# HyeonwooNoh/VQA-Transfer-ExternalData

Measured on AMD Instinct MI355X. Metric: VQA train samples/sec (img+question) at bs512, higher is better.
Workload: dtype f32

## Files before the change

### include/vqa_hot.h

```cpp
#ifndef VQA_HOT_H
#define VQA_HOT_H

#include <stdint.h>

#ifdef __cplusplus
extern "C" {
#endif

#define VQA_HOT_ABI_VERSION 5

enum {
    VQA_OK = 0,
    VQA_ERR_ARG = -1,
    VQA_ERR_ALIGN = -2,
    VQA_ERR_LAUNCH = -3,
    VQA_ERR_UNSUPPORTED = -4,
    VQA_ERR_WORKSPACE = -5
};

int vqa_hot_version(void);
const char* vqa_hot_error_string(int code);

int vqa_gather_features(const float* table, const int32_t* nbox_table, const int64_t* idx,
                        float* V, int32_t* nb, int B, int R, int D, int64_t N, void* stream);
// ... 291 lines not shown
    vqa_fc_t v2l[3];
    vqa_fc_t answer_layer1, pooled_layer1, q_layer1;
    vqa_fc_t classifier;
} vqa_params_t;

typedef struct {
    const float* table;
    const int32_t* nbox_table;
    const int64_t* image_idx;
    const int32_t* q_intseq;
    const int32_t* q_intseq_len;
    const float* answer_target;
    const float *train_mask, *obj_mask, *attr_mask, *exist_mask;
    const uint8_t* keep_att;
    const uint8_t* keep_joint;
    const uint8_t* keep_joint2;
    const int32_t* live_rows;
    const float* noise;
    const uint8_t* keep_tile;
    const uint8_t* keep_word;
    const int32_t* answer_intseq;
    const int32_t* answer_intseq_len;
    uint64_t keep_seed;
    uint64_t keep_att_off, keep_joint_off, keep_joint2_off, keep_tile_off, keep_word_off;
    int32_t keep_seeded;
} vqa_batch_t;
#define VQA_KEEP_SITE_ATT 1
#define VQA_KEEP_SITE_JOINT 2
#define VQA_KEEP_SITE_JOINT2 4
#define VQA_KEEP_SITE_TILE 8
#define VQA_KEEP_SITE_WORD 16

int64_t vqa_fusion_workspace_bytes(const vqa_dims_t* dims);
int vqa_fusion_tensor(const vqa_dims_t* dims, const char* name, int64_t* offset_bytes, int64_t* n_elems);
int vqa_fusion_forward(const vqa_dims_t* dims, const vqa_params_t* params, const vqa_batch_t* batch,
                       void* workspace, int64_t workspace_bytes, int want_dz, void* stream);
int vqa_fusion_backward(const vqa_dims_t* dims, const vqa_params_t* params, const vqa_params_t* grads,
                        const vqa_batch_t* batch, void* workspace, int64_t workspace_bytes,
                        float* embed_slice_sq, void* stream);

typedef struct {
    int32_t B, n, R, D, H, W, A, Vq, n_ws;
    int32_t L;
    int32_t flags;
    float keep_att, keep_joint;
    float global_valid[2];
} vqa_pretrain_dims_t;

typedef struct { float *w, *b, *beta[4], *gamma[4]; } vqa_pt_fc_t;

typedef struct {
    float* wordset_map;
    float* l_glove;
    vqa_pt_fc_t spat_v_linear_v;
    vqa_pt_fc_t spat_q_linear_v;
    vqa_pt_fc_t spat_att_score;
    float *gru_wg, *gru_bg, *gru_wc, *gru_bc;
    vqa_pt_fc_t pooled_linear_l;
    vqa_pt_fc_t q_linear_l;
    vqa_pt_fc_t joint_fc;
    vqa_pt_fc_t wordset_ft;
    vqa_pt_fc_t classifier;
} vqa_pretrain_params_t;

typedef struct {
    const float* normal_boxes;
// ... 290 lines not shown
```

### vqa-transfer-externaldata_amd/_lib.py

```python
from __future__ import annotations

import ctypes as C
import os

_HERE = os.path.dirname(os.path.abspath(__file__))
_LIB_PATH = os.path.join(_HERE, "libvqahot.so")


class VqaHotError(RuntimeError):
    pass


def lib_path():
    return _LIB_PATH


class Dims(C.Structure):
    _fields_ = [("B", C.c_int32), ("R", C.c_int32), ("D", C.c_int32), ("H", C.c_int32), ("T", C.c_int32),
                ("W", C.c_int32), ("A", C.c_int32), ("Vq", C.c_int32), ("N_img", C.c_int64),
                ("model_type", C.c_int32), ("keep_att", C.c_float), ("keep_joint", C.c_float),
                ("inv_global_batch", C.c_float), ("flags", C.c_int32),
                ("num_marginal", C.c_int32), ("ent_cols", C.c_int32), ("extra_weight", C.c_float),
                ("map_dim", C.c_int32), ("La", C.c_int32)]

# ... 184 lines not shown
    "vqa_ln_relu_bwd": (_I, [_P, _P, _P, _P, _P, _P, _P, _F, _P, _P, _P, _P, _I, _I, _I, _P]),
    "vqa_ln_act_fwd": (_I, [_P, _P, _P, _P, _F, _P, _P, _P, _I, _I, _I, _I, _P]),
    "vqa_ln_act_bwd": (_I, [_P, _P, _P, _P, _P, _P, _P, _F, _P, _P, _P, _P, _I, _I, _I, _I, _P]),
    "vqa_ln_pair_mul_supported": (_I, [_I, _P, _I]),
    "vqa_ln_pair_mul_fwd": (_I, [_P] * 13 + [_I, _I, _P]),
    "vqa_ln_pair_mul_bwd": (_I, [_P] * 20 + [_I, _I, _P]),
    "vqa_tanh_fwd": (_I, [_P, _P, _L, _P]),
    "vqa_tanh_bwd": (_I, [_P, _P, _P, _L, _P]),
    "vqa_softmax_ce_fwd": (_I, [_P, _P, _P, _I, _P, _P, _P, _I, _I, _P]),
    "vqa_softmax_set_fast": (_I, [_I]),
    "vqa_softmax_ce_pair_fwd": (_I, [C.POINTER(SoftmaxPair), _I, _I, _I, _I, _P]),
    "vqa_colsum": (_I, [_P, _I, _I, _I, _P, _P, _L, _P]),
    "vqa_colsum_workspace_floats": (_L, [_I, _I]),
    "vqa_colsum3": (_I, [_P, _P, _P, _I, _I, _I, _P, _P, _P, _P, _L, _P]),
    "vqa_colsum_acc": (_I, [_P, _I, _I, _I, _P, _I, _P, _L, _P]),
    "vqa_colsum3_acc": (_I, [_P, _P, _P, _I, _I, _I, _P, _P, _P, _I, _P, _L, _P]),
    "vqa_mul": (_I, [_P, _P, _P, _L, _P]),
    "vqa_mul_bwd": (_I, [_P, _P, _P, _P, _P, _L, _P]),
    "vqa_add_inplace": (_I, [_P, _P, _L, _P]),
    "vqa_gru_gates_fwd": (_I, [_P, _I, _P, _P, _P, _P, _I, _I, _P]),
    "vqa_gru_cand_fwd": (_I, [_P, _I, _P, _P, _P, _I, _P, _P, _I, _I, _P]),
    "vqa_gru_bwd_a": (_I, [_P, _P, _P, _P, _P, _I, _P, _I, _P, _I, _P, _I, _I, _P]),
    "vqa_gru_bwd_b": (_I, [_P, _P, _P, _P, _I, _P, _I, _I, _P]),
    "vqa_attn_set_fast": (_I, [_I]),
    "vqa_attn_pool_fwd": (_I, [_P, _P, _P, _P, _P, _P, _P, _F, _P, _P, _I, _I, _I, _I, _P]),
    "vqa_attn_pool_bwd": (_I, [_P, _P, _P, _P, _P, _P, _P, _F, _P, _P, _P, _P, _I, _I, _I, _I, _P]),
    "vqa_attn_pool_fwd_v16": (_I, [_P, _P, _P, _P, _P, _P, _P, _F, _P, _P, _I, _I, _I, _I, _P]),
    "vqa_attn_pool_bwd_v16": (_I, [_P, _P, _P, _P, _P, _P, _P, _F, _P, _P, _P, _P, _I, _I, _I, _I, _P]),
    "vqa_attn_pool_fwd_rep": (_I, [_P, _P, _P, _P, _P, _P, _P, _F, _P, _P, _I, _I, _I, _I, _I, _P]),
    "vqa_attn_pool_bwd_rep": (_I, [_P, _P, _P, _P, _P, _P, _P, _F, _P, _P, _P, _P, _I, _I, _I, _I, _I, _P]),
    "vqa_vtail_supported": (_I, [_I, _I, _I, _I]),
    "vqa_vtail_set_mode": (_I, [_I]),
    "vqa_gru_h0skip_set_mode": (_I, [_I]),
    "vqa_attn_pool_bwd_ds": (_I, [_P, _P, _P, _P, _P, _I, _I, _I, _I, _I, _P]),
    "vqa_attn_pool_bwd_ds_v16": (_I, [_P, _P, _P, _P, _P, _I, _I, _I, _I, _I, _P]),
    "vqa_ln_relu_att_bwd": (_I, [_P, _P, _P, _P, _F] + [_P] * 11 + [_I, _I, _I, _I, _I, _P]),
    "vqa_attn_pool_fwd_seeded": (_I, [_P, _P, _P, _I, _P, _P, _P, _U, _U, _F, _P, _P, _I, _I, _I, _I, _I, _P]),
    "vqa_attn_pool_bwd_seeded": (_I, [_P, _P, _P, _P, _I, _P, _P, _U, _U, _F, _P, _P, _P, _P, _I, _I, _I, _I, _I, _P]),
    "vqa_attn_pool_fwd_rep_seeded": (_I, [_P, _P, _P, _P, _P, _P, _U, _U, _F, _P, _P, _I, _I, _I, _I, _I, _P]),
    "vqa_attn_pool_bwd_rep_seeded": (_I, [_P, _P, _P, _P, _P, _P, _U, _U, _F, _P, _P, _P, _P, _I, _I, _I, _I, _I, _P]),
    "vqa_ln_act_fwd_seeded": (_I, [_P, _P, _P, _U, _U, _F, _P, _P, _P, _I, _I, _I, _I, _P]),
    "vqa_ln_act_bwd_seeded": (_I, [_P, _P, _P, _P, _P, _P, _U, _U, _F, _P, _P, _P, _P, _I, _I, _I, _I, _P]),
    "vqa_ln_relu_att_bwd_seeded": (_I, [_P, _P, _P, _U, _U, _F] + [_P] * 11 + [_I, _I, _I, _I, _I, _P]),
    "vqa_colsum_vtail_workspace_floats": (_L, [_I, _I]),
    "vqa_colsum_vtail": (_I, [_P] * 5 + [_I, _I] + [_P] * 6 + [_L, _P]),
    "vqa_loss_fwd": (_I, [_P, _P, _P, _P, _P, _P, _I, _F, _P, _P, _P, _I, _I, _P]),
    "vqa_loss2_fwd": (_I, [_P, _P, _P, _P, _P, _P, _P, _F, _P, _P, _P, _P, _P, _I, _I, _I, _P]),
    "vqa_rowmin_mask_fwd": (_I, [_P, _P, _P, _P, _I, _I, _P]),
    "vqa_rowmin_mask_bwd": (_I, [_P, _P, _P, _P, _I, _I, _P]),
    "vqa_report_reduce": (_I, [_P, _I, _P, _P]),
    "vqa_report_key": (C.c_char_p, [_I]),
    "vqa_sumsq": (_I, [_P, _L, _P, _P, _P, _L, _P]),
    "vqa_sumsq_workspace_floats": (_L, [_L]),
    "vqa_clip_adam": (_I, [_P, _P, _P, _P, _L, _P, _F, _F, _F, _F, _F, _P]),
    "vqa_dropout_mask": (_I, [_P, _L, C.c_uint64, C.c_uint64, _F, _P]),
    "vqa_clip_adam_dev": (_I, [_P, _P, _P, _P, _L, _P, _F, _P, _F, _F, _F, _P]),
    "vqa_embed2_fwd": (_I, [_P, _P, _P, _P, _I, _I, _I, _I, _P]),
    "vqa_embed2_bwd": (_I, [_P, _P, _P, _P, _I, _I, _I, _I, _P]),
    "vqa_lstm_step_fwd": (_I, [_P, _P, _P, _P, _I, _P, _P, _I, _I, _P]),
    "vqa_lstm_step_bwd": (_I, [_P, _P, _P, _P, _P, _P, _I, _P, _P, _P, _I, _I, _P]),
    "vqa_relu_fwd": (_I, [_P, _P, _L, _P]),
    "vqa_relu_bwd": (_I, [_P, _P, _P, _L, _P]),
    "vqa_fill": (_I, [_P, _L, _F, _P]),
    "vqa_score_fwd": (_I, [_P, _P, _P, _P, _P, _I, _I, _I, _P]),
    "vqa_score_bwd": (_I, [_P, _P, _P, _P, _P, _P, _P, _I, _I, _I, _P]),
    "vqa_reverse_tokens": (_I, [_P, _P, _P, _I, _I, _P]),
# ... 131 lines not shown
```

### vqa-transfer-externaldata_amd/csrc/fusion_model.hip

```cpp
#include <stdlib.h>
#include <string.h>

#include <string>
#include <vector>

#include "keep_launch.h"

namespace {

struct Entry { const char* name; int64_t off; int64_t n; int esz; };

struct Layout {
    std::vector<Entry> e;
    int64_t total = 0;
    int64_t add(const char* name, int64_t n, int esz = 4) {
        const int64_t off = total;
        e.push_back({name, off, n, esz});
        total += ((n * esz + 255) / 256) * 256;
        return off;
    }
    const Entry* find(const char* name) const {
        for (const auto& x : e)
            if (strcmp(x.name, name) == 0) return &x;
        return nullptr;
    }
};

inline bool has_tuned_head(int mt) { return mt == VQA_MODEL_VQA_ALL2 || mt == VQA_MODEL_VQA_ALL; }
inline bool train_loss_masked(int mt) { return mt != VQA_MODEL_STANDARD; }
inline bool bf16_routed(int mt) { return mt == VQA_MODEL_VLMAP_ANSWER || mt == VQA_MODEL_STANDARD; }
inline bool feat16(const vqa_dims_t& d) { return (d.flags & VQA_FLAG_BF16_FEATURES) != 0; }

void legacy_vqa_layout(Layout& L, const vqa_dims_t& d, int64_t& gw);

Layout make_layout(const vqa_dims_t& d) {
    Layout L;
    const int64_t B = d.B, R = d.R, D = d.D, H = d.H, T = d.T, W = d.W, A = d.A;
    L.add("V_ft", B * R * D, feat16(d) ? 2 : 4);
// ... 151 lines not shown
    int64_t colsum_ws_floats() const { return L.find("colsum_ws")->n; }
};

inline bool env_on(const char* name, bool dflt) {
    const char* e = getenv(name);
    return e == nullptr ? dflt : atoi(e) != 0;
}
inline bool xcat_enabled() { static const bool v = env_on("VQA_HOT_XCAT", true); return v; }
inline bool repack_enabled() { static const bool v = env_on("VQA_HOT_REPACK", false); return v; }
inline bool gru_ws_on() { static const bool v = env_on("VQA_HOT_GRU_WS", true); return v; }
inline bool visual_late_enabled() { static const bool v = env_on("VQA_HOT_VISUAL_LATE", true); return v; }
inline bool ln_pair_enabled() { static const bool v = env_on("VQA_HOT_LN_PAIR", true); return v; }
int g_vtail_mode = -1;
inline int vtail_mode() {
    if (g_vtail_mode < 0) g_vtail_mode = env_on("VQA_HOT_VTAIL", true) ? 1 : 0;
    return g_vtail_mode;
}
int g_h0skip_mode = -1;
inline int h0skip_mode() {
    if (g_h0skip_mode < 0) {
        const char* e = getenv("VQA_HOT_GRU_H0SKIP");
        g_h0skip_mode = e == nullptr ? 1 : (atoi(e) & 3);
    }
    return g_h0skip_mode;
}
int side_max_blocks() {
    static int v = -1;
    if (v < 0) {
        const char* e = getenv("VQA_HOT_SIDE_BLOCKS");
        v = e ? atoi(e) : 0;
    }
    return v;
}
int gather_mode(const vqa_dims_t* dims) {
    static int env = -2;
    if (env == -2) {
        const char* e = getenv("VQA_HOT_GATHER");
        env = e == nullptr ? -1 : (strcmp(e, "fused") == 0 ? 1 : 0);
    }
    if (env >= 0) return env;
    return (dims->flags & VQA_FLAG_FUSED_GATHER) ? 1 : 0;
}

struct Side {
    hipStream_t s = nullptr;
    hipEvent_t fork = nullptr, join = nullptr;
    bool ok = false, tried = false;
};
Side& side_stream() {
    static Side sd[64];
    int dev = 0;
    (void)hipGetDevice(&dev);
    Side& x = sd[dev & 63];
    if (!x.tried) {
        x.tried = true;
        const char* env = getenv("VQA_HOT_OVERLAP");
        if (env != nullptr && env[0] == '1') {
            x.ok = hipStreamCreateWithFlags(&x.s, hipStreamNonBlocking) == hipSuccess &&
                   hipEventCreateWithFlags(&x.fork, hipEventDisableTiming) == hipSuccess &&
                   hipEventCreateWithFlags(&x.join, hipEventDisableTiming) == hipSuccess;
        }
    }
    return x;
}
struct Chains {
    static constexpr int MAXC = 4;
    hipStream_t s[MAXC] = {};
    hipEvent_t fork = nullptr, join[MAXC] = {};
    int n = 1;
    float delay_us = 3.f;
    bool tried = false;
};
Chains& gru_chains() {
    static Chains ch[64];
// ... 321 lines not shown

extern "C" int vqa_fusion_tensor(const vqa_dims_t* dims, const char* name, int64_t* offset_bytes, int64_t* n_elems) {
    if (!dims_ok(dims) || name == nullptr) return VQA_ERR_ARG;
    const Layout L = make_layout(*dims);
    const char* key = name;
    if (strcmp(name, "condition") == 0 && dims->model_type == VQA_MODEL_ANSWER2) key = "q_L_ft2";
    else if (strcmp(name, "condition") == 0 && dims->model_type == VQA_MODEL_BI) key = "q_L_ft";
    else if (dims->model_type == VQA_MODEL_LEGACY_VQA && (strcmp(name, "q_L_ft") == 0 || strcmp(name, "answer_ft") == 0)) {
        const bool q = name[0] == 'q';
        const Entry* hsn = L.find(q ? "lv_hsq" : "lv_hsa");
        const int64_t N = q ? dims->B : dims->A, Tn = q ? dims->T : dims->La;
        if (offset_bytes) *offset_bytes = hsn->off + Tn * N * dims->H * 4;
        if (n_elems) *n_elems = N * dims->H;
        return VQA_OK;
    }
    else if (strcmp(name, "condition") == 0) {
        const Entry* h = L.find("hs");
        if (offset_bytes) *offset_bytes = h->off + (int64_t)dims->T * dims->B * dims->H * 4;
        if (n_elems) *n_elems = (int64_t)dims->B * dims->H;
        return VQA_OK;
    }
    const Entry* e = L.find(key);
    if (e == nullptr) return VQA_ERR_ARG;
    if (offset_bytes) *offset_bytes = e->off;
    if (n_elems) *n_elems = e->n;
    return VQA_OK;
}

extern "C" int vqa_vtail_set_mode(int mode) {
    g_vtail_mode = mode < 0 ? -1 : (mode ? 1 : 0);
    return vtail_mode();
}

extern "C" int vqa_gru_h0skip_set_mode(int mode) {
    g_h0skip_mode = mode < 0 ? -1 : (mode & 3);
    return h0skip_mode();
}

namespace {

struct Step {
    const vqa_dims_t& d;
    const vqa_params_t* const P;
    const vqa_params_t* const G;
    const vqa_batch_t* const bt;
    const Layout L;
    const Ctx c;
    const int mt;
    const int64_t B, R, D, H, T, W, A;
    const int64_t Wp;
    const int64_t Dp;
    Side* sd = nullptr;
    bool forked = false;
    bool fuse_gather = false, visual_late = false;
    const float* q_ft = nullptr;
    const float* qv_in = nullptr;
    const float* lin_in = nullptr;
    bool pair = false;

    Step(const vqa_dims_t* dims, const vqa_params_t* P_, const vqa_params_t* G_, const vqa_batch_t* bt_, void* workspace,
         void* stream)
        : d(*dims), P(P_), G(G_), bt(bt_), L(make_layout(*dims)),
          c{*dims, L, static_cast<char*>(workspace), static_cast<hipStream_t>(stream), 0}, mt(dims->model_type),
          B(dims->B), R(dims->R), D(dims->D), H(dims->H), T(dims->T), W(dims->W), A(dims->A), Wp(x_stride(dims->W)),
          Dp(pooled_dim(*dims)) {}
    Step(const Step&) = delete;
// ... 2 lines not shown
    Ctx side_ctx() const { return Ctx{d, L, c.ws, forked ? sd->s : c.st, forked ? 1 : 0}; }
    const float* hs = nullptr;
    const float* h = nullptr;
    float* dh = nullptr;
    float* dxp = nullptr;
    void bind_bwd() {
        hs = c.f("hs");
        h = hs + T * B * H;
        dh = c.f("d_h0");
        dxp = c.f("dxp");
    }
    const float* Wg_h() const { return P->gru_wg + W * 2 * H; }
    const float* Wc_h() const { return P->gru_wc + W * H; }
};

int side_record(const Step& s) { return !s.forked || join_side_record(*s.sd) ? VQA_OK : VQA_ERR_LAUNCH; }
int side_wait(const Step& s) {
    return !s.forked || hipStreamWaitEvent(s.c.st, s.sd->join, 0) == hipSuccess ? VQA_OK : VQA_ERR_LAUNCH;
}

enum GruForm { GRU_WS, GRU_LIVE, GRU_CHAINS };
enum GruDir { GRU_FWD, GRU_BWD };
GruForm gru_form(GruDir dir, int64_t T, int64_t B, int64_t H, const int32_t* live_rows) {
    const bool ws_ok = gru_ws_on() && (live_rows == nullptr || (T > 0 && live_rows[T - 1] > 0));
    if (ws_ok && (dir == GRU_FWD ? vqa_gru_ws_supported((int)T, (int)B, (int)H) : vqa_gru_ws_bwd_supported((int)T, (int)B, (int)H)) == 1)
        return GRU_WS;
    return live_rows != nullptr ? GRU_LIVE : GRU_CHAINS;
}


void fwd_visual_plan(Step& s) {
    s.sd = &side_stream();
    s.forked = fork_side(s.c, *s.sd);
    s.fuse_gather = !(s.d.flags & VQA_FLAG_BF16_GEMM) && gather_mode(&s.d) == 1 && (s.D % 32 == 0) && (s.H % 4 == 0) &&
                    vqa_aligned16(s.bt->table);
    s.visual_late = !s.forked && visual_late_enabled();
}

int fwd_visual(const Step& s) {
    const Ctx cv = s.side_ctx();
    const vqa_params_t* P = s.P;
    const vqa_batch_t* bt = s.bt;
    const int64_t B = s.B, R = s.R, D = s.D, H = s.H;
    {
        ProbeScope ps("gather", cv.st);
        if (feat16(s.d))
            TRY(vqa_gather_features_bf16(reinterpret_cast<const uint16_t*>(bt->table), bt->nbox_table, bt->image_idx,
                                         cv.u16("V_ft"), cv.i32("num_V_ft"), (int)B, (int)R, (int)D, s.d.N_img, cv.st));
        else
            TRY(vqa_gather_features(bt->table, bt->nbox_table, bt->image_idx, s.fuse_gather ? nullptr : cv.f("V_ft"),
                                    cv.i32("num_V_ft"), (int)B, (int)R, (int)D, s.d.N_img, cv.st));
    }
    if (s.fuse_gather) {
        {
            ProbeScope ps("v_linear_v.fwd_gemm", cv.st);
            TRY(vqa_gemm_f32_gather((int)(B * R), (int)H, (int)D, bt->table, (int)D, bt->image_idx, (int)R, s.d.N_img,
                                    P->v_linear_v.w, (int)H, cv.f("pre_v"), (int)H, P->v_linear_v.b, cv.f("V_ft"), (int)D,
                                    cv.st));
        }
        ProbeScope ps("v_linear_v.ln_fwd", cv.st);
        TRY(vqa_ln_relu_fwd(cv.f("pre_v"), P->v_linear_v.gamma, P->v_linear_v.beta, nullptr, 1.f, cv.f("v_linear_v"),
                            cv.f("mean_v"), cv.f("rstd_v"), (int)B, (int)R, (int)H, cv.st));
    } else {
        TRY(fc_ln_relu_fwd(cv, cv.f("V_ft"), B * R, D, H, P->v_linear_v, (int)R, "pre_v", "v_linear_v", "mean_v", "rstd_v",
                           NO_KEEP, 1.f));
    }
    if (s.mt == VQA_MODEL_ADAPT) {
        VQA_REQUIRE(P->v_adapt.w != nullptr && P->v_adapt.gamma != nullptr, VQA_ERR_ARG);
// ... 622 lines not shown
```

### vqa-transfer-externaldata_amd/csrc/gemm_args.h

```cpp
#pragma once
#include <hip/hip_runtime.h>
#include <stdint.h>

struct GemmArgs {
    int M, N, K;
    const float* A; int lda;
    const float* B; int ldb;
    float* C; int ldc;
    const float* bias;
    const float* D; int ldd;
    int k_per_split;
    int64_t slab_stride;
    int vecA, vecB;
    int tiles_m, tiles_n, nsplit;
    int m_fastest;
    unsigned a_bytes, b_bytes;
    const float* scale;
    int relu;
    int Hi, Wi, Ci, Ho, Wo, cstride, pad_t, pad_l, kw;
    int conv_taps;
    int vec_epi;
    const int64_t* g_idx; int g_R; int64_t g_N; float* g_out; int g_ldo;
};

enum { EPI_PLAIN = 0, EPI_GATES = 1, EPI_CAND = 2, EPI_BWD_RH = 3, EPI_BWD_DH = 4 };
struct EpiArgs {
    int H, t, ldo;
    const int32_t* len;
    const float* h_prev;
    const float* i0;
    const float* i1;
    float* o0;
    float* o1;
    float* o2;
};

GemmArgs vqa_gemm_make_args(int M, int N, int K, const float* A, int lda, const float* B, int ldb, float* C, int ldc,
                            const float* bias, const float* D, int ldd);
int vqa_gru_step_launch(int epi, int cfg, const GemmArgs& a, const EpiArgs& ep, hipStream_t st);
int vqa_gru_rs_launch(int epi, const GemmArgs& a, const EpiArgs& ep, hipStream_t st);
```

### vqa-transfer-externaldata_amd/csrc/gemm_f32.hip

```cpp

#include "vqa_common.h"
#include "gemm_args.h"
#include <cstdio>
#include <cstdlib>

#ifndef VQA_GEMM_STAGGER
#define VQA_GEMM_STAGGER 1
#endif

typedef float f32x16 __attribute__((ext_vector_type(16)));
typedef unsigned int u32x4 __attribute__((ext_vector_type(4)));

#if defined(VQA_DBG_STAMPS)
__device__ unsigned long long* g_dbg_stamps = nullptr;
#define DBG_STAMP(i) do { if (threadIdx.x == 0) dbg_t[i] = __builtin_amdgcn_s_memrealtime(); } while (0)
#else
#define DBG_STAMP(i) do {} while (0)
#endif

namespace {


__device__ __forceinline__ int xcd_remap(int lin, int total) {
    const int q = total >> 3, r = total & 7;
// ... 283 lines not shown
                e_x0[i] = *reinterpret_cast<const float4*>(ep.h_prev + o);
                e_x1[i] = *reinterpret_cast<const float4*>(ep.i0 + o);
                e_x2[i] = *reinterpret_cast<const float4*>(ep.i1 + o);
                e_lim[i] = ep.len[grow];
            }
        }
    }
    float* L0 = smem;
    float* L1 = smem + (A_FL + B_FL);

    if (DEEP == 0) {
        Stager<BM, BK, A_KC, NT> sa;
        Stager<BN, BK, B_KC, NT> sb;
        constexpr int NVA = Stager<BM, BK, A_KC, NT>::NV;
        int iy0[NVA], ix0[NVA], pix[NVA];
        if (CONV) {
#pragma unroll
            for (int i = 0; i < NVA; ++i) {
                const int idx = threadIdx.x + i * NT;
                const int m = m0 + idx / (BK / 4);
                pix[i] = -1; iy0[i] = ix0[i] = 0;
                if (idx < BM * (BK / 4) && m < p.M) {
                    const int hw = p.Ho * p.Wo;
                    const int b = m / hw, r = m - b * hw;
                    const int oy = r / p.Wo, ox = r - oy * p.Wo;
                    iy0[i] = oy * p.cstride - p.pad_t;
                    ix0[i] = ox * p.cstride - p.pad_l;
                    pix[i] = b * p.Hi * p.Wi;
                }
            }
        }
        const float* gsrc[NVA];
        unsigned gdst[NVA];
        const bool g_store = GATHER && p.g_out != nullptr && n0 == 0;
        const __amdgpu_buffer_rsrc_t rsG = __builtin_amdgcn_make_buffer_rsrc(
            p.g_out, 0, GATHER && p.g_out != nullptr ? (int)(((int64_t)(p.M - 1) * p.g_ldo + p.K) * 4) : 0, 0x00020000);
        if (GATHER) {
#pragma unroll
            for (int i = 0; i < NVA; ++i) {
                const int idx = threadIdx.x + i * NT;
                const int row = idx / (BK / 4), kq = (idx % (BK / 4)) * 4;
                const int m = m0 + row, mc = min(m, p.M - 1);
                const int smp = mc / p.g_R, reg_row = mc - smp * p.g_R;
                int64_t src = p.g_idx[smp];
                src = src < 0 ? 0 : (src >= p.g_N ? p.g_N - 1 : src);
                gsrc[i] = p.A + (src * p.g_R + reg_row) * (int64_t)p.lda + kq;
                gdst[i] = (m < p.M) ? (unsigned)(((int64_t)m * p.g_ldo + kq) * 4) : Stager<BM, BK, A_KC, NT>::OOB;
            }
        }
        auto load_a = [&](int k0) {
            if (GATHER) sa.load_ptr(gsrc, k0 - kbeg);
            else if (CONV) sa.load_conv(rsA, iy0, ix0, pix, k0, p.Hi, p.Wi, p.Ci, p.kw);
            else if (EDGE) sa.load(p.A, p.lda, m0, k0, p.M, kend, va);
            else sa.load_fast(rsA, p.lda, m0, k0, p.M, kend);
        };
        auto load_b = [&](int k0) {
            if (EDGE) sb.load(p.B, p.ldb, n0, k0, p.N, kend, vb);
            else sb.load_fast(rsB, p.ldb, n0, k0, p.N, kend);
        };
        if (nt > 0) {
            load_a(kbeg);
            load_b(kbeg);
            sa.store(L0);
            sb.store(L0 + A_FL);
            if (g_store) sa.store_buf(rsG, gdst, 0u);
        }
        __syncthreads();
        int t = 0;
        if (CONV && p.conv_taps <= 32 && p.Ci % BK == 0) {
            unsigned cbase[NVA], cmask[NVA];
            const int kh = p.conv_taps / p.kw;
#pragma unroll
            for (int i = 0; i < NVA; ++i) {
                const int idx = threadIdx.x + i * NT;
                const int kq = (idx % (BK / 4)) * 4;
                cbase[i] = (unsigned)(((int64_t)(pix[i] + iy0[i] * p.Wi + ix0[i]) * p.Ci + kq) * 4);
                unsigned mk = 0;
                if (pix[i] >= 0) {
                    for (int ky = 0; ky < kh; ++ky)
                        for (int kx = 0; kx < p.kw; ++kx)
                            if ((unsigned)(iy0[i] + ky) < (unsigned)p.Hi && (unsigned)(ix0[i] + kx) < (unsigned)p.Wi)
                                mk |= 1u << (ky * p.kw + kx);
                }
                cmask[i] = mk;
            }
            sb.init_full(p.ldb, n0, kbeg, p.N);
            const unsigned stepB = (unsigned)(BK * p.ldb) * 4u;
            unsigned ob = stepB;
            int c0 = BK, ky = 0, kx = 0, tap = 0;
            auto advance = [&]() {
                c0 += BK;
                if (c0 >= p.Ci) { c0 = 0; ++tap; if (++kx == p.kw) { kx = 0; ++ky; } }
            };
            if (c0 >= p.Ci) { c0 = 0; tap = 1; if (++kx == p.kw) { kx = 0; ++ky; } }
            for (; t + 2 < nt; t += 2) {
                sa.load_conv_full(rsA, cbase, cmask, (unsigned)(((ky * p.Wi + kx) * p.Ci + c0) * 4), 1u << tap);
                sb.load_full(rsB, ob);
                ob += stepB; advance();
                __builtin_amdgcn_sched_barrier(0);
                compute_tile(L0, L0 + A_FL);
                __builtin_amdgcn_sched_barrier(0);
                sa.store(L1);
                sb.store(L1 + A_FL);
                __syncthreads();
                sa.load_conv_full(rsA, cbase, cmask, (unsigned)(((ky * p.Wi + kx) * p.Ci + c0) * 4), 1u << tap);
                sb.load_full(rsB, ob);
                ob += stepB; advance();
                __builtin_amdgcn_sched_barrier(0);
                compute_tile(L1, L1 + A_FL);
                __builtin_amdgcn_sched_barrier(0);
                sa.store(L0);
                sb.store(L0 + A_FL);
                __syncthreads();
            }
        }
        if (!CONV && !EDGE) {
            sa.init_full(p.lda, m0, kbeg, p.M);
            sb.init_full(p.ldb, n0, kbeg, p.N);
            const unsigned stepA = (unsigned)(A_KC ? BK : BK * p.lda) * 4u;
            const unsigned stepB = (unsigned)(B_KC ? BK : BK * p.ldb) * 4u;
            const int nfull = (kend - kbeg) / BK;
            unsigned oa = stepA, ob = stepB;
            constexpr bool STAG = (NT == 512) && !GATHER && EPI == EPI_PLAIN && (VQA_GEMM_STAGGER != 0) &&
                                  ((WM == 32 && WN == 32 && BK == 32 && BM + BN == 192) || (BM == 128 && BN == 128 && BK == 16));
            const bool stag_wg = STAG && nfull >= 16;
            if (stag_wg && wave >= 4) {
                sa.load_full(rsA, oa); sb.load_full(rsB, ob);
                oa += stepA; ob += stepB;
                for (; t + 3 < nfull; t += 2) {
                    sa.store(L1); sb.store(L1 + A_FL);
                    sa.load_full(rsA, oa); sb.load_full(rsB, ob);
                    oa += stepA; ob += stepB;
                    __builtin_amdgcn_sched_barrier(0);
                    compute_tile(L0, L0 + A_FL);
                    __builtin_amdgcn_sched_barrier(0);
                    __syncthreads();
                    sa.store(L0); sb.store(L0 + A_FL);
                    sa.load_full(rsA, oa); sb.load_full(rsB, ob);
                    oa += stepA; ob += stepB;
                    __builtin_amdgcn_sched_barrier(0);
                    compute_tile(L1, L1 + A_FL);
                    __builtin_amdgcn_sched_barrier(0);
                    __syncthreads();
                }
                sa.store(L1); sb.store(L1 + A_FL);
                __builtin_amdgcn_sched_barrier(0);
                compute_tile(L0, L0 + A_FL);
                __builtin_amdgcn_sched_barrier(0);
                __syncthreads();
                ++t;
            } else if (stag_wg) {
                for (; t + 3 < nfull; t += 2) {
                    sa.load_full(rsA, oa); sb.load_full(rsB, ob);
                    oa += stepA; ob += stepB;
                    __builtin_amdgcn_sched_barrier(0);
                    compute_tile(L0, L0 + A_FL);
                    __builtin_amdgcn_sched_barrier(0);
                    sa.store(L1); sb.store(L1 + A_FL);
                    __syncthreads();
                    sa.load_full(rsA, oa); sb.load_full(rsB, ob);
                    oa += stepA; ob += stepB;
                    __builtin_amdgcn_sched_barrier(0);
                    compute_tile(L1, L1 + A_FL);
                    __builtin_amdgcn_sched_barrier(0);
                    sa.store(L0); sb.store(L0 + A_FL);
                    __syncthreads();
                }
                sa.load_full(rsA, oa); sb.load_full(rsB, ob);
                __builtin_amdgcn_sched_barrier(0);
                compute_tile(L0, L0 + A_FL);
                __builtin_amdgcn_sched_barrier(0);
                sa.store(L1); sb.store(L1 + A_FL);
                __syncthreads();
                ++t;
            }
            for (; !stag_wg && t + 2 < nfull; t += 2) {
                if (GATHER) sa.load_ptr(gsrc, (t + 1) * BK); else sa.load_full(rsA, oa);
                sb.load_full(rsB, ob);
                oa += stepA; ob += stepB;
                __builtin_amdgcn_sched_barrier(0);
                compute_tile(L0, L0 + A_FL);
                __builtin_amdgcn_sched_barrier(0);
                sa.store(L1);
                sb.store(L1 + A_FL);
                if (g_store) sa.store_buf(rsG, gdst, (unsigned)((t + 1) * BK) * 4u);
                __syncthreads();
                if (GATHER) sa.load_ptr(gsrc, (t + 2) * BK); else sa.load_full(rsA, oa);
                sb.load_full(rsB, ob);
                oa += stepA; ob += stepB;
                __builtin_amdgcn_sched_barrier(0);
                compute_tile(L1, L1 + A_FL);
                __builtin_amdgcn_sched_barrier(0);
                sa.store(L0);
                sb.store(L0 + A_FL);
                if (g_store) sa.store_buf(rsG, gdst, (unsigned)((t + 2) * BK) * 4u);
                __syncthreads();
            }
        }
        for (; t + 1 < nt; ++t) {
            float* cur = (t & 1) ? L1 : L0;
            float* nxt = (t & 1) ? L0 : L1;
            load_a(kbeg + (t + 1) * BK);
            load_b(kbeg + (t + 1) * BK);
            __builtin_amdgcn_sched_barrier(0);
            compute_tile(cur, cur + A_FL);
            __builtin_amdgcn_sched_barrier(0);
            sa.store(nxt);
            sb.store(nxt + A_FL);
            if (g_store) sa.store_buf(rsG, gdst, (unsigned)((t + 1) * BK) * 4u);
            __syncthreads();
        }
        if (nt > 0) {
            float* cur = ((nt - 1) & 1) ? L1 : L0;
            compute_tile(cur, cur + A_FL);
            __syncthreads();
        }
    } else {
        Stager<BM, BK, A_KC, NT> sa0, sa1;
        Stager<BN, BK, B_KC, NT> sb0, sb1;
        auto ld0 = [&](int tile) {
            sa0.load_fast(rsA, p.lda, m0, kbeg + tile * BK, p.M, kend);
            sb0.load_fast(rsB, p.ldb, n0, kbeg + tile * BK, p.N, kend);
        };
        auto ld1 = [&](int tile) {
            sa1.load_fast(rsA, p.lda, m0, kbeg + tile * BK, p.M, kend);
            sb1.load_fast(rsB, p.ldb, n0, kbeg + tile * BK, p.N, kend);
        };
        auto st0 = [&]() { sa0.store(L0); sb0.store(L0 + A_FL); };
        auto st1 = [&]() { sa1.store(L1); sb1.store(L1 + A_FL); };
        if (nt > 0) ld0(0);
        if (nt > 1) ld1(1);
        if (nt > 0) st0();
        __syncthreads();
        DBG_STAMP(1);
        int t = 0;
        {
            sa0.init_full(p.lda, m0, kbeg, p.M); sa1.init_full(p.lda, m0, kbeg, p.M);
            sb0.init_full(p.ldb, n0, kbeg, p.N); sb1.init_full(p.ldb, n0, kbeg, p.N);
#if defined(VQA_DBG_KFREEZE)
            const unsigned stepA = 0, stepB = 0;
#else
            const unsigned stepA = (unsigned)(A_KC ? BK : BK * p.lda) * 4u;
// ... 592 lines not shown
        while (sp > 1 && (workspace == nullptr || workspace_floats < (int64_t)sp * M * N || ldc % 4 != 0 || !vqa_aligned16(C))) sp /= 2;
        return vqa_gemm_bf16x3(transA, M, N, K, A, lda, B, ldb, C, ldc, bias, sp, workspace, workspace_floats, stream);
    }
    if (!transA && !transB && split_k <= 1 && max_blocks == 0 && g_force_cfg < 0 && (shortk_mode() & 1) &&
        M >= 1024 && K <= 304 && vqa_gemm_shortk_supported(M, N, K, lda, ldb, ldc) && !(K > 256 && D != nullptr) && vqa_aligned16(A) &&
        vqa_aligned16(B))
        return vqa_gemm_shortk_nn(M, N, K, A, lda, B, ldb, C, ldc, bias, nullptr, D, ldd, 0, stream);

    int cfg, split = split_k;
    choose(transA, transB, M, N, K, cfg, split);
    if (split > 1 && ((N % 4) != 0 || workspace == nullptr)) split = 1;

    GemmArgs a = vqa_gemm_make_args(M, N, K, A, lda, B, ldb, C, ldc, bias, D, ldd);
    if (split > 1) {
        VQA_REQUIRE(workspace_floats >= (int64_t)split * M * N, VQA_ERR_WORKSPACE);
        int kps = (int)cdiv(cdiv(K, split), 64) * 64;
        a.k_per_split = kps;
        split = (int)cdiv(K, kps);
    }
    if (split > 1) {
        a.C = workspace; a.ldc = N; a.slab_stride = (int64_t)M * N;
        int rc = launch_by_id(cfg, transA, transB, a, split, st, max_blocks);
        if (rc != VQA_OK) return rc;
        const int64_t n4 = (int64_t)M * N / 4;
        const int grid = (int)std::min<int64_t>(cdiv(n4, 256), 2048);
        hipLaunchKernelGGL(splitk_reduce_kernel, dim3(grid), dim3(256), 0, st, workspace, C, M, N, ldc, split);
        VQA_CHECK_LAUNCH();
        return VQA_OK;
    }
    a.k_per_split = (int)cdiv(std::max(K, 1), 64) * 64;
    return launch_by_id(cfg, transA, transB, a, 1, st, max_blocks);
}

extern "C" int vqa_gemm_f32_gather(int M, int N, int K, const float* table, int lda, const int64_t* idx, int R,
                                   int64_t n_samples_in_table, const float* B, int ldb, float* C, int ldc,
                                   const float* bias, float* gathered_out, int ldg, void* stream) {
    VQA_REQUIRE(M >= 0 && N >= 0 && K > 0 && R > 0 && n_samples_in_table > 0, VQA_ERR_ARG);
    if (M == 0 || N == 0) return VQA_OK;
    VQA_REQUIRE(table && idx && B && C, VQA_ERR_ARG);
    VQA_REQUIRE(lda >= K && ldb >= N && ldc >= N && (gathered_out == nullptr || ldg >= K), VQA_ERR_ARG);
    VQA_REQUIRE(K % 32 == 0 && N % 4 == 0, VQA_ERR_UNSUPPORTED);
    VQA_REQUIRE(lda % 4 == 0 && vqa_aligned16(table) && ldb % 4 == 0 && vqa_aligned16(B) &&
                    (gathered_out == nullptr || (ldg % 4 == 0 && vqa_aligned16(gathered_out))),
                VQA_ERR_ALIGN);
    GemmArgs a = vqa_gemm_make_args(M, N, K, table, lda, B, ldb, C, ldc, bias, nullptr, 0);
    const int64_t bb = ((int64_t)(K - 1) * ldb + N) * 4;
    VQA_REQUIRE(bb < 0xFFFFFF00ll, VQA_ERR_UNSUPPORTED);
    a.a_bytes = 0;
    a.b_bytes = (unsigned)bb;
    VQA_REQUIRE(gathered_out == nullptr || ((int64_t)(M - 1) * ldg + K) * 4 < 0xFFFFFF00ll, VQA_ERR_UNSUPPORTED);
    a.g_idx = idx; a.g_R = R; a.g_N = n_samples_in_table; a.g_out = gathered_out; a.g_ldo = ldg;
    a.k_per_split = (int)cdiv(K, 64) * 64;
    const EpiArgs ep{};
    hipStream_t st = static_cast<hipStream_t>(stream);
    if (g_tall_cfg == 21)
        return launch_one<64, 128, 32, 32, 1, 32, 0, true, false, EPI_PLAIN, false, false, 512, true>(a, ep, 1, st, 0);
    return launch_one<128, 64, 32, 32, 1, 32, 0, true, false, EPI_PLAIN, false, false, 512, true>(a, ep, 1, st, 0);
}

extern "C" int vqa_gemm_set_tall_config(int cfg) {
    VQA_REQUIRE(cfg == 20 || cfg == 21, VQA_ERR_ARG);
    g_tall_cfg = cfg;
    return VQA_OK;
}

extern "C" int vqa_conv2d_nhwc(const float* x, int B, int Hi, int Wi, int Ci, const float* w, int kh, int kw, int Co,
                               int stride, int pad_t, int pad_l, int Ho, int Wo, const float* scale,
                               const float* shift, const float* residual, int relu, float* y, void* stream) {
    VQA_REQUIRE(x && w && y && B > 0 && Hi > 0 && Wi > 0 && Ci > 0 && Co > 0 && kh > 0 && kw > 0 && stride > 0 &&
                    Ho > 0 && Wo > 0,
                VQA_ERR_ARG);
    VQA_REQUIRE((int64_t)B * Ho * Wo < (1ll << 31) && (int64_t)B * Hi * Wi < (1ll << 31), VQA_ERR_ARG);
    hipStream_t st = static_cast<hipStream_t>(stream);
    const int M = B * Ho * Wo, K = kh * kw * Ci;
    const bool plain = (kh == 1 && kw == 1 && stride == 1 && pad_t == 0 && pad_l == 0 && Ho == Hi && Wo == Wi);
    GemmArgs a = vqa_gemm_make_args(M, Co, K, x, Ci, w, Co, y, Co, shift, residual, Co);
    a.scale = scale;
    a.relu = relu;
    if (plain && (shortk_mode() & 2) && Ci >= 128 && Ci <= 256 && Co >= 2 * Ci && g_conv_cfg_plain < 0 && g_force_cfg < 0 &&
        vqa_gemm_shortk_supported(M, Co, K, Ci, Co, Co) && vqa_aligned16(x) && vqa_aligned16(w) &&
        (residual == nullptr || (int64_t)M * Co * 4 < 0xFFFFFFF0ll))
// ... 34 lines not shown
```

Measured before the change: 163,900.

## Enable fused gather-GEMM by default via buffer-resource loads when tile config matches

Adds an auto mode that turns on the fused feature-gather GEMM when the table fits in a 32-bit buffer range and the regular GEMM heuristic would pick the same tall tile config. The gather path now loads A through buffer-resource offsets, so it can use the full/staggered pipelined main loop instead of per-pointer loads. This removes a separate gather pass and the extra round trip of the gathered features through memory. The risk is that the fused kernel runs slower than the plain GEMM path, or that the gathered-output writes added to every loop variant slow down the inner loop.

```diff
diff --git a/include/vqa_hot.h b/include/vqa_hot.h
--- a/include/vqa_hot.h
+++ b/include/vqa_hot.h
@@ -347,6 +347,8 @@
 #define VQA_KEEP_SITE_WORD 16
 
 int64_t vqa_fusion_workspace_bytes(const vqa_dims_t* dims);
+int vqa_fusion_gather_fused(const vqa_dims_t* dims);
+int vqa_gather_set_mode(int mode);
 int vqa_fusion_tensor(const vqa_dims_t* dims, const char* name, int64_t* offset_bytes, int64_t* n_elems);
 int vqa_fusion_forward(const vqa_dims_t* dims, const vqa_params_t* params, const vqa_batch_t* batch,
                        void* workspace, int64_t workspace_bytes, int want_dz, void* stream);
diff --git a/vqa-transfer-externaldata_amd/_lib.py b/vqa-transfer-externaldata_amd/_lib.py
--- a/vqa-transfer-externaldata_amd/_lib.py
+++ b/vqa-transfer-externaldata_amd/_lib.py
@@ -240,6 +240,8 @@
     "vqa_vtail_supported": (_I, [_I, _I, _I, _I]),
     "vqa_vtail_set_mode": (_I, [_I]),
     "vqa_gru_h0skip_set_mode": (_I, [_I]),
+    "vqa_gather_set_mode": (_I, [_I]),
+    "vqa_fusion_gather_fused": (_I, [_P]),
     "vqa_attn_pool_bwd_ds": (_I, [_P, _P, _P, _P, _P, _I, _I, _I, _I, _I, _P]),
     "vqa_attn_pool_bwd_ds_v16": (_I, [_P, _P, _P, _P, _P, _I, _I, _I, _I, _I, _P]),
     "vqa_ln_relu_att_bwd": (_I, [_P, _P, _P, _P, _F] + [_P] * 11 + [_I, _I, _I, _I, _I, _P]),
diff --git a/vqa-transfer-externaldata_amd/csrc/fusion_model.hip b/vqa-transfer-externaldata_amd/csrc/fusion_model.hip
--- a/vqa-transfer-externaldata_amd/csrc/fusion_model.hip
+++ b/vqa-transfer-externaldata_amd/csrc/fusion_model.hip
@@ -4,6 +4,7 @@
 #include <string>
 #include <vector>
 
+#include "gemm_args.h"
 #include "keep_launch.h"
 
 namespace {
@@ -221,14 +222,25 @@
     }
     return v;
 }
+enum { GATHER_PASS = 0, GATHER_FUSED = 1, GATHER_AUTO = 2 };
+int g_gather_mode = -1;
 int gather_mode(const vqa_dims_t* dims) {
+    if (g_gather_mode >= 0) return g_gather_mode ? GATHER_FUSED : GATHER_PASS;
     static int env = -2;
     if (env == -2) {
         const char* e = getenv("VQA_HOT_GATHER");
-        env = e == nullptr ? -1 : (strcmp(e, "fused") == 0 ? 1 : 0);
+        env = e == nullptr ? -1 : (strcmp(e, "fused") == 0 ? GATHER_FUSED : GATHER_PASS);
     }
     if (env >= 0) return env;
-    return (dims->flags & VQA_FLAG_FUSED_GATHER) ? 1 : 0;
+    return (dims->flags & VQA_FLAG_FUSED_GATHER) ? GATHER_FUSED : GATHER_AUTO;
+}
+bool gather_fused(const vqa_dims_t& d) {
+    if ((d.flags & VQA_FLAG_BF16_GEMM) || d.D % 32 != 0 || d.H % 4 != 0) return false;
+    if (d.model_type == VQA_MODEL_LEGACY_VQA) return false;
+    const int mode = gather_mode(&d);
+    if (mode != GATHER_AUTO) return mode == GATHER_FUSED;
+    const bool small_table = ((int64_t)d.N_img * d.R * d.D) * 4 < 0xFFFFFF00ll;
+    return small_table && vqa_gemm_gather_same_tile((int)((int64_t)d.B * d.R), (int)d.H, (int)d.D);
 }
 
 struct Side {
@@ -616,6 +628,17 @@
     return vtail_mode();
 }
 
+extern "C" int vqa_gather_set_mode(int mode) {
+    g_gather_mode = mode < 0 ? -1 : (mode > 2 ? 1 : mode);
+    vqa_gemm_gather_set_wide(g_gather_mode == 2);
+    return g_gather_mode;
+}
+
+extern "C" int vqa_fusion_gather_fused(const vqa_dims_t* dims) {
+    VQA_REQUIRE(dims != nullptr && dims_ok(dims), VQA_ERR_ARG);
+    return gather_fused(*dims) ? 1 : 0;
+}
+
 extern "C" int vqa_gru_h0skip_set_mode(int mode) {
     g_h0skip_mode = mode < 0 ? -1 : (mode & 3);
     return h0skip_mode();
@@ -684,8 +707,7 @@
 void fwd_visual_plan(Step& s) {
     s.sd = &side_stream();
     s.forked = fork_side(s.c, *s.sd);
-    s.fuse_gather = !(s.d.flags & VQA_FLAG_BF16_GEMM) && gather_mode(&s.d) == 1 && (s.D % 32 == 0) && (s.H % 4 == 0) &&
-                    vqa_aligned16(s.bt->table);
+    s.fuse_gather = gather_fused(s.d) && vqa_aligned16(s.bt->table);
     s.visual_late = !s.forked && visual_late_enabled();
 }
 
diff --git a/vqa-transfer-externaldata_amd/csrc/gemm_args.h b/vqa-transfer-externaldata_amd/csrc/gemm_args.h
--- a/vqa-transfer-externaldata_amd/csrc/gemm_args.h
+++ b/vqa-transfer-externaldata_amd/csrc/gemm_args.h
@@ -37,5 +37,7 @@
 
 GemmArgs vqa_gemm_make_args(int M, int N, int K, const float* A, int lda, const float* B, int ldb, float* C, int ldc,
                             const float* bias, const float* D, int ldd);
+bool vqa_gemm_gather_same_tile(int M, int N, int K);
+void vqa_gemm_gather_set_wide(bool on);
 int vqa_gru_step_launch(int epi, int cfg, const GemmArgs& a, const EpiArgs& ep, hipStream_t st);
 int vqa_gru_rs_launch(int epi, const GemmArgs& a, const EpiArgs& ep, hipStream_t st);
diff --git a/vqa-transfer-externaldata_amd/csrc/gemm_f32.hip b/vqa-transfer-externaldata_amd/csrc/gemm_f32.hip
--- a/vqa-transfer-externaldata_amd/csrc/gemm_f32.hip
+++ b/vqa-transfer-externaldata_amd/csrc/gemm_f32.hip
@@ -339,6 +339,7 @@
         }
         const float* gsrc[NVA];
         unsigned gdst[NVA];
+        const bool g32 = GATHER && p.a_bytes != 0;
         const bool g_store = GATHER && p.g_out != nullptr && n0 == 0;
         const __amdgpu_buffer_rsrc_t rsG = __builtin_amdgcn_make_buffer_rsrc(
             p.g_out, 0, GATHER && p.g_out != nullptr ? (int)(((int64_t)(p.M - 1) * p.g_ldo + p.K) * 4) : 0, 0x00020000);
@@ -351,12 +352,20 @@
                 const int smp = mc / p.g_R, reg_row = mc - smp * p.g_R;
                 int64_t src = p.g_idx[smp];
                 src = src < 0 ? 0 : (src >= p.g_N ? p.g_N - 1 : src);
-                gsrc[i] = p.A + (src * p.g_R + reg_row) * (int64_t)p.lda + kq;
-                gdst[i] = (m < p.M) ? (unsigned)(((int64_t)m * p.g_ldo + kq) * 4) : Stager<BM, BK, A_KC, NT>::OOB;
-            }
-        }
+                const int64_t roff = (src * p.g_R + reg_row) * (int64_t)p.lda + kq;
+                gsrc[i] = p.A + roff;
+                sa.voff[i] = (unsigned)(roff * 4);
+                gdst[i] = (g_store && m < p.M) ? (unsigned)(((int64_t)m * p.g_ldo + kq) * 4) : Stager<BM, BK, A_KC, NT>::OOB;
+            }
+        }
+        auto g_put = [&](int tile) {
+            sa.store_buf(rsG, gdst, (unsigned)(tile * BK) * 4u);
+        };
         auto load_a = [&](int k0) {
-            if (GATHER) sa.load_ptr(gsrc, k0 - kbeg);
+            if (GATHER) {
+                if (g32) sa.load_full(rsA, (unsigned)(k0 - kbeg) * 4u);
+                else sa.load_ptr(gsrc, k0 - kbeg);
+            }
             else if (CONV) sa.load_conv(rsA, iy0, ix0, pix, k0, p.Hi, p.Wi, p.Ci, p.kw);
             else if (EDGE) sa.load(p.A, p.lda, m0, k0, p.M, kend, va);
             else sa.load_fast(rsA, p.lda, m0, k0, p.M, kend);
@@ -370,7 +379,7 @@
             load_b(kbeg);
             sa.store(L0);
             sb.store(L0 + A_FL);
-            if (g_store) sa.store_buf(rsG, gdst, 0u);
+            if (GATHER) g_put(0);
         }
         __syncthreads();
         int t = 0;
@@ -421,14 +430,14 @@
                 __syncthreads();
             }
         }
-        if (!CONV && !EDGE) {
-            sa.init_full(p.lda, m0, kbeg, p.M);
+        if (!CONV && !EDGE && (!GATHER || g32)) {
+            if (!GATHER) sa.init_full(p.lda, m0, kbeg, p.M);
             sb.init_full(p.ldb, n0, kbeg, p.N);
             const unsigned stepA = (unsigned)(A_KC ? BK : BK * p.lda) * 4u;
             const unsigned stepB = (unsigned)(B_KC ? BK : BK * p.ldb) * 4u;
             const int nfull = (kend - kbeg) / BK;
             unsigned oa = stepA, ob = stepB;
-            constexpr bool STAG = (NT == 512) && !GATHER && EPI == EPI_PLAIN && (VQA_GEMM_STAGGER != 0) &&
+            constexpr bool STAG = (NT == 512) && EPI == EPI_PLAIN && (VQA_GEMM_STAGGER != 0) &&
                                   ((WM == 32 && WN == 32 && BK == 32 && BM + BN == 192) || (BM == 128 && BN == 128 && BK == 16));
             const bool stag_wg = STAG && nfull >= 16;
             if (stag_wg && wave >= 4) {
@@ -436,6 +445,7 @@
                 oa += stepA; ob += stepB;
                 for (; t + 3 < nfull; t += 2) {
                     sa.store(L1); sb.store(L1 + A_FL);
+                    if (GATHER) g_put(t + 1);
                     sa.load_full(rsA, oa); sb.load_full(rsB, ob);
                     oa += stepA; ob += stepB;
                     __builtin_amdgcn_sched_barrier(0);
@@ -443,6 +453,7 @@
                     __builtin_amdgcn_sched_barrier(0);
                     __syncthreads();
                     sa.store(L0); sb.store(L0 + A_FL);
+                    if (GATHER) g_put(t + 2);
                     sa.load_full(rsA, oa); sb.load_full(rsB, ob);
                     oa += stepA; ob += stepB;
                     __builtin_amdgcn_sched_barrier(0);
@@ -451,6 +462,7 @@
                     __syncthreads();
                 }
                 sa.store(L1); sb.store(L1 + A_FL);
+                if (GATHER) g_put(t + 1);
                 __builtin_amdgcn_sched_barrier(0);
                 compute_tile(L0, L0 + A_FL);
                 __builtin_amdgcn_sched_barrier(0);
@@ -464,6 +476,7 @@
                     compute_tile(L0, L0 + A_FL);
                     __builtin_amdgcn_sched_barrier(0);
                     sa.store(L1); sb.store(L1 + A_FL);
+                    if (GATHER) g_put(t + 1);
                     __syncthreads();
                     sa.load_full(rsA, oa); sb.load_full(rsB, ob);
                     oa += stepA; ob += stepB;
@@ -471,6 +484,7 @@
                     compute_tile(L1, L1 + A_FL);
                     __builtin_amdgcn_sched_barrier(0);
                     sa.store(L0); sb.store(L0 + A_FL);
+                    if (GATHER) g_put(t + 2);
                     __syncthreads();
                 }
                 sa.load_full(rsA, oa); sb.load_full(rsB, ob);
@@ -478,11 +492,12 @@
                 compute_tile(L0, L0 + A_FL);
                 __builtin_amdgcn_sched_barrier(0);
                 sa.store(L1); sb.store(L1 + A_FL);
+                if (GATHER) g_put(t + 1);
                 __syncthreads();
                 ++t;
             }
             for (; !stag_wg && t + 2 < nfull; t += 2) {
-                if (GATHER) sa.load_ptr(gsrc, (t + 1) * BK); else sa.load_full(rsA, oa);
+                sa.load_full(rsA, oa);
                 sb.load_full(rsB, ob);
                 oa += stepA; ob += stepB;
                 __builtin_amdgcn_sched_barrier(0);
@@ -490,9 +505,9 @@
                 __builtin_amdgcn_sched_barrier(0);
                 sa.store(L1);
                 sb.store(L1 + A_FL);
-                if (g_store) sa.store_buf(rsG, gdst, (unsigned)((t + 1) * BK) * 4u);
+                if (GATHER) g_put(t + 1);
                 __syncthreads();
-                if (GATHER) sa.load_ptr(gsrc, (t + 2) * BK); else sa.load_full(rsA, oa);
+                sa.load_full(rsA, oa);
                 sb.load_full(rsB, ob);
                 oa += stepA; ob += stepB;
                 __builtin_amdgcn_sched_barrier(0);
@@ -500,7 +515,34 @@
                 __builtin_amdgcn_sched_barrier(0);
                 sa.store(L0);
                 sb.store(L0 + A_FL);
-                if (g_store) sa.store_buf(rsG, gdst, (unsigned)((t + 2) * BK) * 4u);
+                if (GATHER) g_put(t + 2);
+                __syncthreads();
+            }
+        } else if (GATHER) {
+            sb.init_full(p.ldb, n0, kbeg, p.N);
+            const unsigned stepB = (unsigned)(B_KC ? BK : BK * p.ldb) * 4u;
+            const int nfull = (kend - kbeg) / BK;
+            unsigned ob = stepB;
+            for (; t + 2 < nfull; t += 2) {
+                sa.load_ptr(gsrc, (t + 1) * BK);
+                sb.load_full(rsB, ob);
+                ob += stepB;
+                __builtin_amdgcn_sched_barrier(0);
+                compute_tile(L0, L0 + A_FL);
+                __builtin_amdgcn_sched_barrier(0);
+                sa.store(L1);
+                sb.store(L1 + A_FL);
+                if (g_store) g_put(t + 1);
+                __syncthreads();
+                sa.load_ptr(gsrc, (t + 2) * BK);
+                sb.load_full(rsB, ob);
+                ob += stepB;
+                __builtin_amdgcn_sched_barrier(0);
+                compute_tile(L1, L1 + A_FL);
+                __builtin_amdgcn_sched_barrier(0);
+                sa.store(L0);
+                sb.store(L0 + A_FL);
+                if (g_store) g_put(t + 2);
                 __syncthreads();
             }
         }
@@ -514,7 +556,7 @@
             __builtin_amdgcn_sched_barrier(0);
             sa.store(nxt);
             sb.store(nxt + A_FL);
-            if (g_store) sa.store_buf(rsG, gdst, (unsigned)((t + 1) * BK) * 4u);
+            if (GATHER) g_put(t + 1);
             __syncthreads();
         }
         if (nt > 0) {
@@ -1173,6 +1215,18 @@
     return launch_by_id(cfg, transA, transB, a, 1, st, max_blocks);
 }
 
+bool vqa_gemm_gather_same_tile(int M, int N, int K) {
+    if (M <= 0 || N <= 0 || K <= 0 || g_force_cfg >= 0) return false;
+    if (bf16x3_mode() || ((shortk_mode() & 1) && K <= 304)) return false;
+    if ((int64_t)M * K * 4 >= 0xFFFFFF00ll || (int64_t)K * N * 4 >= 0xFFFFFF00ll || K % 32 != 0 || N % 4 != 0) return false;
+    int cfg, split = 0;
+    choose(0, 0, M, N, K, cfg, split);
+    return cfg == g_tall_cfg && split == 1 && (cfg == 20 || cfg == 21);
+}
+
+bool g_gather_wide = false;
+void vqa_gemm_gather_set_wide(bool on) { g_gather_wide = on; }
+
 extern "C" int vqa_gemm_f32_gather(int M, int N, int K, const float* table, int lda, const int64_t* idx, int R,
                                    int64_t n_samples_in_table, const float* B, int ldb, float* C, int ldc,
                                    const float* bias, float* gathered_out, int ldg, void* stream) {
@@ -1187,7 +1241,8 @@
     GemmArgs a = vqa_gemm_make_args(M, N, K, table, lda, B, ldb, C, ldc, bias, nullptr, 0);
     const int64_t bb = ((int64_t)(K - 1) * ldb + N) * 4;
     VQA_REQUIRE(bb < 0xFFFFFF00ll, VQA_ERR_UNSUPPORTED);
-    a.a_bytes = 0;
+    const int64_t tb = ((n_samples_in_table * R - 1) * (int64_t)lda + K) * 4;
+    a.a_bytes = (!g_gather_wide && tb < 0xFFFFFF00ll) ? (unsigned)tb : 0u;
     a.b_bytes = (unsigned)bb;
     VQA_REQUIRE(gathered_out == nullptr || ((int64_t)(M - 1) * ldg + K) * 4 < 0xFFFFFF00ll, VQA_ERR_UNSUPPORTED);
     a.g_idx = idx; a.g_R = R; a.g_N = n_samples_in_table; a.g_out = gathered_out; a.g_ldo = ldg;
```

Result: no change. 165,200 (median of 6 runs) (+0.8%).
